# HandBrake/HandBrake

Measured on AMD Instinct MI355X. Metric: filtered frames/sec, 1080p YUV420p NLMeans+decomb chain, higher is better.
Workload: dtype u8 (f32 NLMeans weights, 16-bit fixed-point scaler as zimg, sharpen mix = the reference's f64 expression, as one f32 multiply where init proves that equal); 1 GPU; BASELINE configs[3]: decomb(31, EEDI2 bob) -> nlmeans medium -> cropscale lanczos 1920x1080 -> 3840x2160 -> lapsharp, 1080i YUV420P 8-bit in, inputs resident in HBM; input=1920x1080, output=3840x2160, streams_per_gpu=1, content=interlaced, stream_frames=48, stage_streams=2, parallelism=1 GPU(s) x 1 independent stream(s), device=AMD Radeon Graphics (gfx950:sramecc+:xnack-, 256 CUs)

## Files before the change

### handbrake_amd/csrc/decomb.hip

```cpp
#include "hbhip_internal.h"
#include "eedi2_engine.h"
#include <algorithm>
#include <vector>

namespace {

enum { M_YADIF = 1, M_BLEND = 2, M_CUBIC = 4, M_EEDI2 = 8, M_BOB = 16, M_SELECTIVE = 32 };
enum { PIC_TFF = 0x0008, PIC_PROGRESSIVE = 0x0010 };

struct DecombPlane
{
    const uint8_t *prev, *cur, *next, *guess;
    uint8_t       *dst;
    int            pitch, guess_pitch, dst_pitch, w, h;
};

struct DecombArgs
{
    DecombPlane pl[3];
    int mode;
    int parity;
    int field_parity;
};

// ... 5 lines not shown
__device__ __forceinline__ int max3i(int a, int b, int c) { return max(max(a, b), c); }
__device__ __forceinline__ int min3i(int a, int b, int c) { return min(min(a, b), c); }

constexpr int DB_FRAMES = 16;

struct DecombFrame
{
    const uint8_t *prev[3], *cur[3], *next[3], *guess[3];
    uint8_t       *dst[3];
    int mode, parity, field_parity, pad;
};

struct DecombBatch
{
    DecombFrame f[DB_FRAMES];
    int pitch[3], guess_pitch[3], dst_pitch[3], w[3], h[3];
    int n = 0;
    int ff = 0;
};

template <typename PIX> struct Px4;
template <> struct Px4<uint8_t>
{
    typedef uint32_t T;
    static __device__ __forceinline__ T zero() { return 0u; }
    static __device__ __forceinline__ int get(T v, int k) { return (int)((v >> (8 * k)) & 0xffu); }
    static __device__ __forceinline__ T pack(const int (&o)[4]) { return ((uint32_t)o[0] & 0xffu) | (((uint32_t)o[1] & 0xffu) << 8) | (((uint32_t)o[2] & 0xffu) << 16) | ((uint32_t)o[3] << 24); }
};
template <> struct Px4<uint16_t>
{
    typedef uint2 T;
    static __device__ __forceinline__ T zero() { return make_uint2(0u, 0u); }
    static __device__ __forceinline__ int get(T v, int k) { return (int)(((k < 2 ? v.x : v.y) >> (16 * (k & 1))) & 0xffffu); }
    static __device__ __forceinline__ T pack(const int (&o)[4]) { return make_uint2(((uint32_t)o[0] & 0xffffu) | ((uint32_t)o[1] << 16), ((uint32_t)o[2] & 0xffffu) | ((uint32_t)o[3] << 16)); }
};
template <typename PIX> struct W12 { typename Px4<PIX>::T w0, w1, w2; };

template <typename PIX>
__device__ __forceinline__ int w12b(const W12<PIX> &w, int i)
{
    const int k = i + 4;
    return Px4<PIX>::get(k < 4 ? w.w0 : (k < 8 ? w.w1 : w.w2), k & 3);
}

template <typename PIX>
__device__ __forceinline__ W12<PIX> ldw12(const uint8_t *row, int x, int pitch)
{
    typedef typename Px4<PIX>::T T;
    const T *p = reinterpret_cast<const T *>(row + (size_t)x * sizeof(PIX));
    return W12<PIX>{ x >= 4 ? p[-1] : Px4<PIX>::zero(), p[0], x + 4 < pitch ? p[1] : Px4<PIX>::zero() };
}

template <typename PIX>
__global__ __launch_bounds__(256) void decomb_plane4_kernel(DecombBatch B, int maxv)
{
    typedef Px4<PIX> X4;
    typedef typename X4::T T;
    typedef W12<PIX> WIN;
    const int pl = blockIdx.z % 3;
    const DecombFrame &F = B.f[blockIdx.z / 3];
    const int w = B.w[pl], h = B.h[pl], st = B.pitch[pl];
    const int pitch_s = st / (int)sizeof(PIX);
    const int x = 4 * (blockIdx.x * blockDim.x + threadIdx.x);
    const int y = blockIdx.y * blockDim.y + threadIdx.y;
    if (x >= w || y >= h) return;
    const uint8_t *cb = F.cur[pl];
    const uint8_t *crow = cb + (size_t)y * st;
    uint8_t *orow = F.dst[pl] + (size_t)y * B.dst_pitch[pl];
    const int mode = F.mode;
    auto store = [&](T v) {
        PIX *o = reinterpret_cast<PIX *>(orow) + x;
        if (x + 3 < w) *reinterpret_cast<T *>(o) = v;
        else for (int k = 0; k < 4 && x + k < w; k++) o[k] = (PIX)X4::get(v, k);
    };
    auto dw = [&](const uint8_t *row) { return *reinterpret_cast<const T *>(row + (size_t)x * sizeof(PIX)); };
    auto dwb = [](T v, int k) { return X4::get(v, k); };

    if (mode == 0) { store(dw(crow)); return; }
    if ((mode & M_EEDI2) && !(mode & M_YADIF))
    {
        store(dw(F.guess[pl] + (size_t)y * B.guess_pitch[pl]));
        return;
    }
    if ((y & 1) != (F.parity ? 0 : 1)) { store(dw(crow)); return; }

    int o4[4] = { 0, 0, 0, 0 };
    if (mode == M_BLEND)
    {
        int u1, u2, d1, d2;
        if (y > 1 && y < h - 2) { u1 = -st; u2 = -2 * st; d1 = st; d2 = 2 * st; }
        else if (y == 0)        { u1 = u2 = 0; d1 = st; d2 = 2 * st; }
        else if (y == 1)        { u1 = u2 = -st; d1 = st; d2 = 2 * st; }
        else if (y == h - 2)    { u1 = -st; u2 = -2 * st; d1 = d2 = st; }
        else                    { u1 = -st; u2 = -2 * st; d1 = d2 = 0; }
        const T a2 = dw(crow + u2), a1 = dw(crow + u1), c0 = dw(crow), b1 = dw(crow + d1), b2 = dw(crow + d2);
#pragma unroll
        for (int k = 0; k < 4; k++)
            o4[k] = cropv((-dwb(a2, k) + 2 * dwb(a1, k) + 6 * dwb(c0, k) + 2 * dwb(b1, k) - dwb(b2, k)) >> 3, maxv);
        store(X4::pack(o4));
        return;
    }
    if (mode == M_CUBIC)
    {
        int o0, o1, o2, o3;
        if (y >= 3)                { o0 = -3 * st; o1 = -st; }
        else if (y == 2 || y == 1) { o0 = o1 = -st; }
        else                       { o0 = o1 = st; }
        if (y <= h - 4)                    { o2 = st; o3 = 3 * st; }
        else if (y == h - 3 || y == h - 2) { o2 = o3 = st; }
        else                               { o2 = o3 = -st; }
        const T p0 = dw(crow + o0), p1 = dw(crow + o1), p2 = dw(crow + o2), p3 = dw(crow + o3);
#pragma unroll
        for (int k = 0; k < 4; k++) o4[k] = cubic4(dwb(p0, k), dwb(p1, k), dwb(p2, k), dwb(p3, k), maxv);
        store(X4::pack(o4));
        return;
    }
    if (!(mode & M_YADIF)) return;

// ... 48 lines not shown
        const int td2 = (abs(dwb(pnu, k) - cc) + abs(dwb(pnd, k) - e)) >> 1;
        int diff = max3i(td0 >> 1, td1, td2);
        int pred;
        if (!spatial) pred = dwb(g, k);
        else
        {
            pred = use_cubic ? cubic4(w12b(cu3, k), cc, e, w12b(cd3, k), maxv) : (cc + e) >> 1;
            const int xx = x + k;
            if (xx > margin && xx < w - (margin + 1))
            {
                auto slope = [&](int j) -> int {
                    if constexpr (sizeof(PIX) == 1)
                        return (int)__builtin_amdgcn_sad_u8(CU[3 + k + j], CD[3 + k - j], 0u);
                    else
                        return abs(w12b(cu, k - 1 + j) - w12b(cd, k - 1 - j)) + abs(w12b(cu, k + j) - w12b(cd, k - j)) +
                               abs(w12b(cu, k + 1 + j) - w12b(cd, k + 1 - j));
                };
                int best = slope(0) - 1;
                auto check = [&](int j) -> bool {
                    const int score = slope(j);
                    if (score >= best) return false;
                    best = score;
                    if (use_cubic)
                    {
                        if (j == -1)      pred = cubic4(w12b(cu3, k - 3), w12b(cu, k - 1), w12b(cd, k + 1), w12b(cd3, k + 3), maxv);
                        else if (j == -2) pred = cubic4((w12b(cu3, k - 4) + w12b(cu, k - 4)) / 2, w12b(cu, k - 2), w12b(cd, k + 2),
                                                        (w12b(cd3, k + 4) + w12b(cd, k + 4)) / 2, maxv);
                        else if (j == 1)  pred = cubic4(w12b(cu3, k + 3), w12b(cu, k + 1), w12b(cd, k - 1), w12b(cd3, k - 3), maxv);
                        else              pred = cubic4((w12b(cu3, k + 4) + w12b(cu, k + 4)) / 2, w12b(cu, k + 2), w12b(cd, k - 2),
                                                        (w12b(cd3, k - 4) + w12b(cd, k - 4)) / 2, maxv);
                    }
                    else pred = (w12b(cu, k + j) + w12b(cd, k - j)) >> 1;
                    return true;
                };
                if (check(-1)) check(-2);
                if (check(1)) check(2);
            }
        }
        if (!vertical_edge)
        {
            const int b = (dwb(p2a, k) + dwb(n2a, k)) >> 1;
            const int f = (dwb(p2b, k) + dwb(n2b, k)) >> 1;
            const int mx = max3i(d - e, d - cc, min(b - cc, f - e));
            const int mn = min3i(d - e, d - cc, max(b - cc, f - e));
            diff = max3i(diff, mn, -mx);
        }
        if (pred > d + diff)      pred = d + diff;
        else if (pred < d - diff) pred = d - diff;
        o4[k] = pred;
    }
    store(X4::pack(o4));
}


template <typename PIX>
__global__ __launch_bounds__(256) void bwdif_kernel(DecombArgs a, int field_end, int clip_max)
{
    typedef Px4<PIX> X4;
    typedef typename X4::T T;
    const DecombPlane &P = a.pl[blockIdx.z];
    const int x = 4 * (blockIdx.x * blockDim.x + threadIdx.x);
    const int y = blockIdx.y * blockDim.y + threadIdx.y;
    if (x >= P.w || y >= P.h) return;
    const int st = P.pitch, df = (int)sizeof(PIX), h = P.h;
    const uint8_t *cur = P.cur + (size_t)y * st;
    uint8_t *orow = P.dst + (size_t)y * P.dst_pitch;
    auto dw = [&](const uint8_t *row) { return *reinterpret_cast<const T *>(row + (size_t)x * sizeof(PIX)); };
    auto store = [&](T v) {
        PIX *o = reinterpret_cast<PIX *>(orow) + x;
        if (x + 3 < P.w) *reinterpret_cast<T *>(o) = v;
        else for (int k = 0; k < 4 && x + k < P.w; k++) o[k] = (PIX)X4::get(v, k);
    };
    if (a.mode == 0 || !((y ^ a.parity) & 1))
    {
        store(dw(cur));
        return;
    }
    constexpr int lf0 = 4309, lf1 = 213, hf0 = 5570, hf1 = 3801, hf2 = 1016, sp0 = 5077, sp1 = 981;
    int o4[4];
    if (field_end)
    {
        const int prefs = (y + df) < h ? st : -st, mrefs = y > (df - 1) ? -st : st;
        const int prefs3 = (y + 3 * df) < h ? 3 * st : -st, mrefs3 = y > (3 * df - 1) ? -3 * st : st;
        const T c1 = dw(cur + mrefs), e1 = dw(cur + prefs), c3 = dw(cur + mrefs3), e3 = dw(cur + prefs3);
#pragma unroll
        for (int k = 0; k < 4; k++)
        {
            const int v = (sp0 * (X4::get(c1, k) + X4::get(e1, k)) - sp1 * (X4::get(c3, k) + X4::get(e3, k))) >> 13;
            o4[k] = min(max(v, 0), clip_max);
        }
        store(X4::pack(o4));
        return;
    }
    const uint8_t *prev = P.prev + (size_t)y * st, *next = P.next + (size_t)y * st;
    const uint8_t *prev2 = a.field_parity ? prev : cur;
    const uint8_t *next2 = a.field_parity ? cur : next;
    const bool edge = (y < 4) || ((y + 5) > h);
    const int prefs = edge ? ((y + df) < h ? st : -st) : st, mrefs = edge ? (y > (df - 1) ? -st : st) : -st;
    const bool spat = edge ? !((y < 2) || ((y + 3) > h)) : true;
    const T wc = dw(cur + mrefs), we = dw(cur + prefs), wp0 = dw(prev2), wn0 = dw(next2);
    const T wpm = dw(prev + mrefs), wpp = dw(prev + prefs), wnm = dw(next + mrefs), wnp = dw(next + prefs);
    T wp2a = X4::zero(), wn2a = X4::zero(), wp2b = X4::zero(), wn2b = X4::zero();
    if (spat) { wp2a = dw(prev2 - 2 * st); wn2a = dw(next2 - 2 * st); wp2b = dw(prev2 + 2 * st); wn2b = dw(next2 + 2 * st); }
    T wc3a = X4::zero(), wc3b = X4::zero(), wp4a = X4::zero(), wn4a = X4::zero(), wp4b = X4::zero(), wn4b = X4::zero();
    if (!edge)
    {
// ... 171 lines not shown
        DecombArgs a;
        for (int c = 0; c < 3; c++)
        {
            DecombPlane &P = a.pl[c];
            P.prev = ref[0]->plane[c]; P.cur = ref[1]->plane[c]; P.next = ref[2]->plane[c];
            P.guess = nullptr; P.guess_pitch = 0;
            if ((mode & M_EEDI2) && eedi && slot >= 0)
            {
                const EediFrame g = eedi->result(slot);
                P.guess = g.plane[c];
                P.guess_pitch = g.stride[c];
            }
            P.dst = dst->plane[c];
            P.pitch = ref[1]->pitch[c]; P.dst_pitch = dst->pitch[c];
            P.w = in_geo.pw[c]; P.h = in_geo.ph[c];
        }
        a.mode = mode; a.parity = parity; a.field_parity = parity ^ tff;
        dim3 block(64, 4), grid((in_geo.pw[0] + 63) / 64, (in_geo.ph[0] + 3) / 4, 3);
        const int maxv = (1 << in_geo.depth) - 1;
        if (ff_bwdif)
        {
            if (bw_second && bw_field == BW_BACK_END) bw_field = BW_END;
            const int field_end = mode != 0 && bw_field == BW_END;
            const dim3 grid4(hbhip_grid_x((in_geo.pw[0] + 255) / 256), (in_geo.ph[0] + 3) / 4, 3);
            if (in_geo.bps == 2) HBHIP_LAUNCH(ctx, "bwdif", bwdif_kernel<uint16_t>, grid4, block, 0, a, field_end, maxv);
            else                 HBHIP_LAUNCH(ctx, "bwdif", bwdif_kernel<uint8_t>, grid4, block, 0, a, field_end, maxv);
            if (mode != 0 && bw_field == BW_END) bw_field = BW_NORMAL;
            HBHIP_CHECK(ctx, hipGetLastError());
            return HBHIP_OK;
        }
        geo.ff = ff_yadif ? (ff_nospatial ? 2 : 1) : 0;
        DecombFrame F;
        for (int c = 0; c < 3; c++)
        {
            const DecombPlane &P = a.pl[c];
            F.prev[c] = P.prev; F.cur[c] = P.cur; F.next[c] = P.next; F.guess[c] = P.guess; F.dst[c] = P.dst;
            geo.pitch[c] = P.pitch; geo.dst_pitch[c] = P.dst_pitch; geo.w[c] = P.w; geo.h[c] = P.h;
            if (P.guess) geo.guess_pitch[c] = P.guess_pitch;
        }
        F.mode = a.mode; F.parity = a.parity; F.field_parity = a.field_parity; F.pad = 0;
        gathered.push_back(F);
        return HBHIP_OK;
    }

    int launch_gathered(hbhip_ctx *lc)
    {
        for (size_t i0 = 0; i0 < gathered.size(); i0 += DB_FRAMES)
        {
            DecombBatch B = geo;
            B.n = (int)std::min<size_t>(DB_FRAMES, gathered.size() - i0);
            for (int k = 0; k < B.n; k++) B.f[k] = gathered[i0 + k];
            const dim3 block(64, 4), grid(hbhip_grid_x((B.w[0] + 255) / 256), (B.h[0] + 3) / 4, 3 * B.n);
            const int maxv = (1 << in_geo.depth) - 1;
            if (ff_yadif)
            {
                if (in_geo.bps == 2) HBHIP_LAUNCH(lc, "yadif", decomb_plane4_kernel<uint16_t>, grid, block, 0, B, maxv);
                else                 HBHIP_LAUNCH(lc, "yadif", decomb_plane4_kernel<uint8_t>, grid, block, 0, B, maxv);
            }
            else
            {
                if (in_geo.bps == 2) HBHIP_LAUNCH(lc, "decomb_plane", decomb_plane4_kernel<uint16_t>, grid, block, 0, B, maxv);
                else                 HBHIP_LAUNCH(lc, "decomb_plane", decomb_plane4_kernel<uint8_t>, grid, block, 0, B, maxv);
            }
        }
        const bool any = !gathered.empty();
        gathered.clear();
        if (any) HBHIP_CHECK(lc, hipGetLastError());
        return HBHIP_OK;
    }

    int process_frame()
    {
        DevPicture *cur = ref[1];
        const bool selective = par.mode & M_SELECTIVE;
        if (selective && cur->combed == 0)
        {
            DevPicture *o = pool.acquire();
            if (!o) return HBHIP_ERR_NOMEM;
            o->tag = cur->tag << 1; o->aux = 0;
            bw_second = false;
            int rc = launch(o, 0, 0, 0);
            if (rc != HBHIP_OK) return rc;
            outq.push_back(o);
            return HBHIP_OK;
        }
        int tff;
        if (par.parity < 0)
            tff = ff_yadif ? (cur->combed ? !!(cur->flags & PIC_TFF) : 1)
                           : (((cur->flags & PIC_PROGRESSIVE) == 0) ? !!(cur->flags & PIC_TFF) : 1);
        else
            tff = (par.parity & 1) ^ 1;

        const int is_combed = selective ? cur->combed : 2;
        int mode = 0;
        if ((par.mode & M_BLEND) && is_combed == 1) mode = M_BLEND;
        else if (is_combed != 0)                    mode = par.mode & ~M_SELECTIVE;

        const int nframes = (par.mode & M_BOB) ? 2 : 1;
        for (int frame = 0; frame < nframes; frame++)
        {
            const int parity = frame ^ tff ^ 1;
            int slot = -1;
            if ((mode & M_EEDI2) && eedi)
            {
                if (eedi->queued() == eedi->capacity())
                {
                    int rc = flush_batch();
// ... 140 lines not shown
```

### handbrake_amd/csrc/sharpen.hip

```cpp
#include <map>
#include <mutex>
#include <utility>
#include "hbhip_internal.h"

namespace {

struct LapKernel { int tap[25]; int size; double coef; };

constexpr LapKernel LAP_TABLE[4] = {
    { { 0, -1, 0, -1, 5, -1, 0, -1, 0 }, 3, 1.0 },
    { { -1, -4, -1, -4, 25, -4, -1, -4, -1 }, 3, 1.0 / 5 },
    { { 0, 0, -1, 0, 0, 0, -1, -2, -1, 0, -1, -2, 21, -2, -1, 0, -1, -2, -1, 0, 0, 0, -1, 0, 0 }, 5, 1.0 / 5 },
    { { 0, -1, -1, -1, 0, -1, -3, -4, -3, -1, -1, -4, 55, -4, -1, -1, -3, -4, -3, -1, 0, -1, -1, -1, 0 }, 5, 1.0 / 15 } };

struct LapArgs
{
    const uint8_t *src;
    uint8_t       *dst;
    int            width, height, src_pitch, dst_pitch;
    int            stride_border;
    int            valid_w;
    int            tap[25];
    double         coef, strength;
};

struct LapArgs3 { LapArgs p[3]; };

__device__ __forceinline__ uint32_t byte_at(const uint32_t (&v)[3], int k)
{
    const int kk = k + 4;
    return (v[kk >> 2] >> (8 * (kk & 3))) & 0xffu;
}

template <int S>
__global__ __launch_bounds__(256) void lapsharp_kernel(LapArgs3 all)
{
    const LapArgs &a = all.p[blockIdx.z];
    constexpr int LO = -((S - 1) / 2), HI = (S + 1) / 2;
    const int x0 = (blockIdx.x * blockDim.x + threadIdx.x) * 4;
    const int y = blockIdx.y;
    if (x0 >= a.width || y >= a.height) return;

    const int pitch_dw = a.src_pitch >> 2;
    const int xd = x0 >> 2;
    uint32_t rows[S][3];
#pragma unroll
    for (int j = 0; j < S; j++)
    {
        int yy = y + LO + j;
        yy = min(max(yy, 0), a.height - 1);
        const uint32_t *r = reinterpret_cast<const uint32_t *>(a.src + (size_t)yy * a.src_pitch);
        rows[j][0] = r[max(xd - 1, 0)];
        rows[j][1] = r[xd];
        rows[j][2] = r[min(xd + 1, pitch_dw - 1)];
        if (x0 + 8 > a.valid_w)
        {
// ... 409 lines not shown
            const uint32_t t = (uint32_t)tf;
            const int p = (int)((C[S] >> (8 * k)) & 0xffu);
            const int blur = (int)((t + (uint32_t)P.halfscale) >> P.scalebits);
            const int d = ((p - blur) * P.amount) >> 16;
            int res = B.sign > 0 ? p + d : p - d;
            res = res > B.vmax ? B.vmax : res < B.vmin ? B.vmin : res;
            packed |= (uint32_t)res << (8 * k);
        }
        store_row(y, packed);
#pragma unroll
        for (int j = 0; j < NT - 1; j++)
        {
            C[j] = C[j + 1];
#pragma unroll
            for (int k = 0; k < 4; k++) H[j][k] = H[j + 1][k];
        }
    }
}

__global__ void plane_copy_kernel(uint8_t *dst, int dst_pitch, const uint8_t *src, int src_pitch,
                                  int row_bytes, int rows)
{
    const int x = (blockIdx.x * blockDim.x + threadIdx.x) * 4;
    const int y = blockIdx.y;
    if (y >= rows || x >= row_bytes) return;
    const uint8_t *s = src + (size_t)y * src_pitch + x;
    uint8_t *d = dst + (size_t)y * dst_pitch + x;
    if (x + 3 < row_bytes)
        *reinterpret_cast<uint32_t *>(d) = *reinterpret_cast<const uint32_t *>(s);
    else
        for (int i = 0; x + i < row_bytes; i++) d[i] = s[i];
}

int launch_copy(hbhip_ctx *ctx, const char *name, DevPicture *in, DevPicture *out, int c)
{
    const int row = in->width[c] * in->bps;
    dim3 grid((row / 4 + 255) / 256 + 1, in->height[c]);
    HBHIP_LAUNCH(ctx, name, plane_copy_kernel, grid, dim3(256), 0, out->plane[c], out->pitch[c],
                 (const uint8_t *)in->plane[c], in->pitch[c], row, in->height[c]);
    HBHIP_CHECK(ctx, hipGetLastError());
    return HBHIP_OK;
}

#ifndef LS_ROWS_N
#define LS_ROWS_N 8
#endif
#ifndef LS_BX_N
#define LS_BX_N 64
#endif
#ifndef LS_ROWS16_N
#define LS_ROWS16_N 4
#endif
constexpr int LS_ROWS = LS_ROWS_N, LS_ROWS16 = LS_ROWS16_N, LS_FRAMES = 16, LS_BX = LS_BX_N, LS_BY = 256 / LS_BX_N;
struct LapPlane3 { int width, height, src_pitch, dst_pitch, stride_border, valid_w, a, b, c, active; double coef, strength; int fast, kinv; float mixf; };
struct LapBatch3
{
    LapPlane3      pl[3];
    const uint8_t *src[LS_FRAMES][3];
    uint8_t       *dst[LS_FRAMES][3];
};

__global__ __launch_bounds__(256) void lapsharp3_rows_kernel(LapBatch3 B)
{
    const int job = blockIdx.z, f = job / 3, c = job - 3 * f;
    const LapPlane3 &P = B.pl[c];
    if (!P.active) return;
    const int x0 = (blockIdx.x * LS_BX + threadIdx.x) * 4;
    const int ys = (blockIdx.y * LS_BY + threadIdx.y) * LS_ROWS;
    if (x0 >= P.width || ys >= P.height) return;
    const uint8_t *src = B.src[f][c];
    uint8_t *dst = B.dst[f][c];
    const int pitch_dw = P.src_pitch >> 2, xd = x0 >> 2;
    const bool tail = x0 + 8 > P.valid_w;

    int u_prev[4], u_cur[4], v_cur[4], m_cur[4];
    const uint32_t o0 = 4u * (uint32_t)max(xd - 1, 0), o1 = 4u * (uint32_t)xd, o2 = 4u * (uint32_t)min(xd + 1, pitch_dw - 1);
    uint32_t raw[LS_ROWS + 2][3];
#pragma unroll
    for (int i = 0; i < LS_ROWS + 2; i++)
    {
        const int yy = min(max(ys - 1 + i, 0), P.height - 1);
        const uint32_t ro = (uint32_t)__mul24(yy, P.src_pitch);
        raw[i][0] = *reinterpret_cast<const uint32_t *>(src + (ro + o0));
        raw[i][1] = *reinterpret_cast<const uint32_t *>(src + (ro + o1));
        raw[i][2] = *reinterpret_cast<const uint32_t *>(src + (ro + o2));
    }
    auto load_row = [&](int i, int (&u)[4], int (&v)[4], int (&m)[4]) {
        uint32_t w[3] = { raw[i][0], raw[i][1], raw[i][2] };
        if (tail)
        {
#pragma unroll
            for (int k = 0; k < 3; k++)
            {
                const int keep = P.valid_w - (x0 - 4 + 4 * k);
                if (keep <= 0) w[k] = 0;
                else if (keep < 4) w[k] &= (1u << (8 * keep)) - 1u;
            }
        }
        const int b_1 = (int)(w[0] >> 24), b0 = (int)(w[1] & 0xff), b1 = (int)((w[1] >> 8) & 0xff),
                  b2 = (int)((w[1] >> 16) & 0xff), b3 = (int)(w[1] >> 24), b4 = (int)(w[2] & 0xff);
        const int bb[6] = { b_1, b0, b1, b2, b3, b4 };
#pragma unroll
        for (int k = 0; k < 4; k++)
        {
            const int h = bb[k] + bb[k + 2];
            m[k] = bb[k + 1];
            u[k] = __mul24(P.a, h) + __mul24(P.b, m[k]);
// ... 14 lines not shown
#pragma unroll
    for (int r = 0; r < LS_ROWS; r++)
    {
        const int y = ys + r;
        if (y >= y_end) break;
        int u_next[4], v_next[4], m_next[4];
        load_row(r + 2, u_next, v_next, m_next);
        const bool row_copy = (y < 2) || (y > P.height - 2);
        uint32_t packed = 0;
        if (row_copy)
        {
#pragma unroll
            for (int k = 0; k < 4; k++) packed |= (uint32_t)m_cur[k] << (8 * k);
        }
        else
        {
            if (P.fast)
            {
#pragma unroll
                for (int k = 0; k < 4; k++)
                {
                    const int centre = m_cur[k];
                    const int acc = u_prev[k] + v_cur[k] + u_next[k];
                    int out = (int)((float)(acc - __mul24(P.kinv, centre)) * P.mixf) + centre;
                    out = min(max(out, 0), 255);
                    packed |= (uint32_t)out << (8 * k);
                }
            }
            else
            {
#pragma unroll
                for (int k = 0; k < 4; k++)
                {
                    const int centre = m_cur[k];
                    const int acc = u_prev[k] + v_cur[k] + u_next[k];
                    const double mixed = (((double)acc * P.coef) - (double)centre) * P.strength;
                    int out = (int)(short)(int)mixed + centre;
                    out = min(max(out, 0), 255);
                    packed |= (uint32_t)out << (8 * k);
                }
            }
            if (copy_cols)
            {
#pragma unroll
                for (int k = 0; k < 4; k++)
                    if ((copy_cols >> k) & 1u) packed = (packed & ~(0xffu << (8 * k))) | ((uint32_t)m_cur[k] << (8 * k));
            }
        }
        uint8_t *d = dst + ((uint32_t)__mul24(y, P.dst_pitch) + (uint32_t)x0);
        if (full_dword) *reinterpret_cast<uint32_t *>(d) = packed;
        else for (int k = 0; x0 + k < P.width; k++) d[k] = (uint8_t)(packed >> (8 * k));
#pragma unroll
        for (int k = 0; k < 4; k++) { u_prev[k] = u_cur[k]; u_cur[k] = u_next[k]; v_cur[k] = v_next[k]; m_cur[k] = m_next[k]; }
    }
}

__global__ __launch_bounds__(256) void lapsharp3_rows16_kernel(LapBatch3 B, int max_value)
{
    const int job = blockIdx.z, f = job / 3, c = job - 3 * f;
    const LapPlane3 &P = B.pl[c];
    if (!P.active) return;
    const int x0 = (blockIdx.x * LS_BX + threadIdx.x) * 4;
    const int ys = (blockIdx.y * LS_BY + threadIdx.y) * LS_ROWS16;
    if (x0 >= P.width || ys >= P.height) return;
    const uint8_t *src = B.src[f][c];
    uint8_t *dst = B.dst[f][c];
    const int pitch_dw = P.src_pitch >> 2, xd = x0 >> 1;
    const bool tail = x0 + 5 > P.width;
    const uint32_t o0 = 4u * (uint32_t)max(xd - 1, 0), o1 = 4u * (uint32_t)xd, o2 = 4u * (uint32_t)min(xd + 1, pitch_dw - 1),
                   o3 = 4u * (uint32_t)min(xd + 2, pitch_dw - 1);
    int u_prev[4], u_cur[4], v_cur[4], m_cur[4];
    uint32_t raw[LS_ROWS16 + 2][4];
#pragma unroll
    for (int i = 0; i < LS_ROWS16 + 2; i++)
    {
        const uint32_t ro = (uint32_t)__mul24(min(max(ys - 1 + i, 0), P.height - 1), P.src_pitch);
        raw[i][0] = *reinterpret_cast<const uint32_t *>(src + (ro + o0)); raw[i][1] = *reinterpret_cast<const uint32_t *>(src + (ro + o1));
        raw[i][2] = *reinterpret_cast<const uint32_t *>(src + (ro + o2)); raw[i][3] = *reinterpret_cast<const uint32_t *>(src + (ro + o3));
    }
    auto load_row = [&](int i, int (&u)[4], int (&v)[4], int (&m)[4]) {
        const uint32_t ro = (uint32_t)__mul24(min(max(ys - 1 + i, 0), P.height - 1), P.src_pitch);
        const uint32_t w0 = raw[i][0], w1 = raw[i][1], w2 = raw[i][2], w3 = raw[i][3];
        int bb[6] = { (int)(w0 >> 16), (int)(w1 & 0xffffu), (int)(w1 >> 16), (int)(w2 & 0xffffu), (int)(w2 >> 16), (int)(w3 & 0xffffu) };
        if (tail)
        {
            const uint16_t *r16 = reinterpret_cast<const uint16_t *>(src + ro);
#pragma unroll
            for (int k = 0; k < 6; k++)
            {
                const int xx = x0 - 1 + k;
                if (xx >= P.width) bb[k] = (int)r16[max(2 * P.width - 1 - xx, 0)];
            }
        }
#pragma unroll
        for (int k = 0; k < 4; k++)
        {
            const int h = bb[k] + bb[k + 2];
            m[k] = bb[k + 1];
            u[k] = __mul24(P.a, h) + __mul24(P.b, m[k]);
            v[k] = __mul24(P.b, h) + __mul24(P.c, m[k]);
        }
    };
    {
        int v_tmp[4], m_tmp[4];
        load_row(0, u_prev, v_tmp, m_tmp);
        load_row(1, u_cur, v_cur, m_cur);
// ... 54 lines not shown
                if ((int)(short)(int)mixed != (int)prod) { ok = false; break; }
            }
        if (ok) { kinv = ki; mixf = c; return true; }
    }
    return false;
}

static bool lap_float_mix_cached(int kernel, double strength, int &kinv, float &mixf)
{
    struct Entry { bool ok; int kinv; float mixf; };
    static std::mutex lock;
    static std::map<std::pair<int, double>, Entry> cache;
    std::lock_guard<std::mutex> lk(lock);
    const auto key = std::make_pair(kernel, strength);
    auto it = cache.find(key);
    if (it == cache.end())
    {
        Entry e = { false, 0, 0.f };
        e.ok = lap_float_mix(LAP_TABLE[kernel], strength, e.kinv, e.mixf);
        it = cache.emplace(key, e).first;
    }
    kinv = it->second.kinv;
    mixf = it->second.mixf;
    return it->second.ok;
}

class LapsharpFilter : public BurstFilter
{
public:
    LapsharpFilter(hbhip_ctx *c, const hbhip_lapsharp_params &p) : BurstFilter(c), par(p)
    {
        for (int pl = 0; pl < 3; pl++)
        {
            mix_fast[pl] = LAP_TABLE[par.kernel[pl]].size == 3 && lap_float_mix_cached(par.kernel[pl], par.strength[pl], mix_k[pl], mix_f[pl]);
            rows3 &= LAP_TABLE[par.kernel[pl]].size == 3;
        }
    }
    template <class P>
    void fill_plane(P &p, const DevPicture *in, const DevPicture *out, int c) const
    {
        p.width = in->width[c]; p.height = in->height[c];
        p.src_pitch = in->pitch[c]; p.dst_pitch = out->pitch[c];
        const int hb_stride = in_is_dev ? hbhip_align_up(in->width[c] * in->bps, 64) / in->bps : in_stride[c] / in->bps;
        p.stride_border = (hb_stride - in->width[c]) / 2;
        p.valid_w = in_is_dev ? in->width[c] : (1 << 30);
        p.coef = LAP_TABLE[par.kernel[c]].coef; p.strength = par.strength[c];
    }
    int process_many(DevPicture *const *ins, DevPicture *const *outs, int n) override
    {
        return hbhip_for_each_run(ctx, ins, outs, n, LS_FRAMES, [&](int at, int nf) {
            if (!rows3) return hbhip_each_frame(ins, outs, at, nf, [&](DevPicture *in, DevPicture *out) { return one_frame(in, out); });
            LapBatch3 B;
            int max_w = 0, max_h = 0;
            for (int c = 0; c < 3; c++)
            {
                const LapKernel &k = LAP_TABLE[par.kernel[c]];
                LapPlane3 &P = B.pl[c];
                fill_plane(P, ins[at], outs[at], c);
                P.a = k.tap[0]; P.b = k.tap[1]; P.c = k.tap[4];
                P.active = 1;
                P.fast = in_geo.bps == 1 && mix_fast[c]; P.kinv = mix_k[c]; P.mixf = mix_f[c];
                max_w = std::max(max_w, P.width); max_h = std::max(max_h, P.height);
                for (int f = 0; f < nf; f++)
                {
                    B.src[f][c] = ins[at + f]->plane[c];
                    B.dst[f][c] = outs[at + f]->plane[c];
                }
            }
            const int rows = LS_BY * (in_geo.bps == 1 ? LS_ROWS : LS_ROWS16);
            const dim3 grid(hbhip_grid_x(((max_w + 3) / 4 + LS_BX - 1) / LS_BX), (max_h + rows - 1) / rows, 3 * nf);
            if (in_geo.bps == 1) HBHIP_LAUNCH(ctx, "lapsharp_3x3", lapsharp3_rows_kernel, grid, dim3(LS_BX, LS_BY), 0, B);
            else                 HBHIP_LAUNCH(ctx, "lapsharp_3x3", lapsharp3_rows16_kernel, grid, dim3(LS_BX, LS_BY), 0, B, (1 << in_geo.depth) - 1);
            return HBHIP_OK;
        });
    }
    int one_frame(DevPicture *in, DevPicture *out)
    {
        for (int size : {3, 5})
        {
            LapArgs3 all;
            int n = 0, max_w = 0, max_h = 0;
            for (int c = 0; c < 3; c++)
            {
                const LapKernel &k = LAP_TABLE[par.kernel[c]];
                if (k.size != size) continue;
                LapArgs &a = all.p[n++];
                a.src = in->plane[c]; a.dst = out->plane[c];
                fill_plane(a, in, out, c);
                for (int i = 0; i < 25; i++) a.tap[i] = k.tap[i];
                max_w = std::max(max_w, a.width); max_h = std::max(max_h, a.height);
            }
            if (n == 0) continue;
            const char *name = size == 3 ? "lapsharp_3x3" : "lapsharp_5x5";
            if (in->bps == 2)
            {
                const dim3 grid(((max_w + 1) / 2 + 255) / 256, max_h, n);
                const int max_value = (1 << in_geo.depth) - 1;
                if (size == 3) HBHIP_LAUNCH(ctx, name, lapsharp16_kernel<3>, grid, dim3(256), 0, all, max_value);
                else           HBHIP_LAUNCH(ctx, name, lapsharp16_kernel<5>, grid, dim3(256), 0, all, max_value);
            }
            else
            {
                const dim3 grid(((max_w + 3) / 4 + 255) / 256, max_h, n);
                if (size == 3) HBHIP_LAUNCH(ctx, name, lapsharp_kernel<3>, grid, dim3(256), 0, all);
                else           HBHIP_LAUNCH(ctx, name, lapsharp_kernel<5>, grid, dim3(256), 0, all);
            }
        }
        return HBHIP_OK;
    }
    hbhip_lapsharp_params par;
    bool  rows3 = true;
    bool  mix_fast[3] = {};
    int   mix_k[3] = {};
    float mix_f[3] = {};
};

static void binomial_row(int steps, uint32_t *coef, int len)
{
    for (int i = 0; i < len; i++) coef[i] = 0;
    coef[0] = 1;
// ... 148 lines not shown
```

Measured before the change: 9792 output frames/s.

## Add row-walking decomb EEDI2+yadif kernel and wide DPP/udot4 lapsharp kernel

Adds a decomb kernel where each thread walks several field rows of the EEDI2+yadif path, keeping cur/prev/next and temporal rows in registers and also writing the copied field line. This cuts redundant global loads and per-row setup. Separately, adds a wide 3x3 lapsharp kernel that covers 8 pixels per thread, shares horizontal neighbours across lanes via DPP, and computes row sums with udot4/alignbyte. Both are gated by runtime checks (8-bit input, tap signs, alignment) and fall back to the old kernels otherwise. The price is higher register pressure and fewer threads in flight.

```diff
diff --git a/handbrake_amd/csrc/decomb.hip b/handbrake_amd/csrc/decomb.hip
--- a/handbrake_amd/csrc/decomb.hip
+++ b/handbrake_amd/csrc/decomb.hip
@@ -81,18 +81,13 @@
 }
 
 template <typename PIX>
-__global__ __launch_bounds__(256) void decomb_plane4_kernel(DecombBatch B, int maxv)
+__device__ __forceinline__ void decomb_row4(const DecombBatch &B, const DecombFrame &F, int pl, int x, int y, int maxv)
 {
     typedef Px4<PIX> X4;
     typedef typename X4::T T;
     typedef W12<PIX> WIN;
-    const int pl = blockIdx.z % 3;
-    const DecombFrame &F = B.f[blockIdx.z / 3];
     const int w = B.w[pl], h = B.h[pl], st = B.pitch[pl];
     const int pitch_s = st / (int)sizeof(PIX);
-    const int x = 4 * (blockIdx.x * blockDim.x + threadIdx.x);
-    const int y = blockIdx.y * blockDim.y + threadIdx.y;
-    if (x >= w || y >= h) return;
     const uint8_t *cb = F.cur[pl];
     const uint8_t *crow = cb + (size_t)y * st;
     uint8_t *orow = F.dst[pl] + (size_t)y * B.dst_pitch[pl];
@@ -247,6 +242,95 @@
     store(X4::pack(o4));
 }
 
+template <typename PIX>
+__global__ __launch_bounds__(256) void decomb_plane4_kernel(DecombBatch B, int maxv)
+{
+    const int pl = blockIdx.z % 3;
+    const int x = 4 * (blockIdx.x * blockDim.x + threadIdx.x);
+    const int y = blockIdx.y * blockDim.y + threadIdx.y;
+    if (x >= B.w[pl] || y >= B.h[pl]) return;
+    decomb_row4<PIX>(B, B.f[blockIdx.z / 3], pl, x, y, maxv);
+}
+
+#ifndef DW_R_N
+#define DW_R_N 8
+#endif
+constexpr int DW_R = DW_R_N;
+
+__global__ __launch_bounds__(256) void decomb_rowwalk8_kernel(DecombBatch B, int maxv)
+{
+    typedef Px4<uint8_t> X4;
+    const int pl = blockIdx.z % 3;
+    const DecombFrame &F = B.f[blockIdx.z / 3];
+    const int w = B.w[pl], h = B.h[pl], st = B.pitch[pl], dst_st = B.dst_pitch[pl];
+    const int x = 4 * (blockIdx.x * blockDim.x + threadIdx.x);
+    const int ys = (blockIdx.y * blockDim.y + threadIdx.y) * (2 * DW_R);
+    if (x >= w || ys >= h) return;
+    const int y0 = ys + (F.parity ? 0 : 1);
+    const bool walk = (F.mode & M_EEDI2) && (F.mode & M_YADIF) && !B.ff && y0 >= 3 && y0 + 2 * (DW_R - 1) <= h - 4;
+    if (!walk)
+    {
+        for (int r = 0; r < 2 * DW_R && ys + r < h; r++) decomb_row4<uint8_t>(B, F, pl, x, ys + r, maxv);
+        return;
+    }
+    auto dw = [&](const uint8_t *base, int y, int pitch) { return *reinterpret_cast<const uint32_t *>(base + (size_t)y * pitch + x); };
+    auto store = [&](int y, uint32_t v) {
+        uint8_t *o = F.dst[pl] + (size_t)y * dst_st + x;
+        if (x + 3 < w) *reinterpret_cast<uint32_t *>(o) = v;
+        else for (int k = 0; k < 4 && x + k < w; k++) o[k] = (uint8_t)X4::get(v, k);
+    };
+    const uint8_t *p2base = F.field_parity ? F.prev[pl] : F.cur[pl], *n2base = F.field_parity ? F.cur[pl] : F.next[pl];
+    uint32_t cu[DW_R + 1], pv[DW_R + 1], nx[DW_R + 1], p2[DW_R + 2], n2[DW_R + 2], gs[DW_R];
+#pragma unroll
+    for (int i = 0; i < DW_R + 1; i++)
+    {
+        cu[i] = dw(F.cur[pl], y0 - 1 + 2 * i, st); pv[i] = dw(F.prev[pl], y0 - 1 + 2 * i, st); nx[i] = dw(F.next[pl], y0 - 1 + 2 * i, st);
+    }
+#pragma unroll
+    for (int i = 0; i < DW_R + 2; i++) { p2[i] = dw(p2base, y0 - 2 + 2 * i, st); n2[i] = dw(n2base, y0 - 2 + 2 * i, st); }
+#pragma unroll
+    for (int i = 0; i < DW_R; i++) gs[i] = dw(F.guess[pl], y0 + 2 * i, B.guess_pitch[pl]);
+
+    int cc[4], a_pu[4], a_nu[4], b[4], d[4], td0[4];
+#pragma unroll
+    for (int k = 0; k < 4; k++)
+    {
+        cc[k] = X4::get(cu[0], k);
+        a_pu[k] = abs(X4::get(pv[0], k) - cc[k]);
+        a_nu[k] = abs(X4::get(nx[0], k) - cc[k]);
+        b[k] = (X4::get(p2[0], k) + X4::get(n2[0], k)) >> 1;
+        d[k] = (X4::get(p2[1], k) + X4::get(n2[1], k)) >> 1;
+        td0[k] = abs(X4::get(p2[1], k) - X4::get(n2[1], k));
+    }
+#pragma unroll
+    for (int i = 0; i < DW_R; i++)
+    {
+        const int y = y0 + 2 * i;
+        int o4[4];
+#pragma unroll
+        for (int k = 0; k < 4; k++)
+        {
+            const int e = X4::get(cu[i + 1], k);
+            const int a_pd = abs(X4::get(pv[i + 1], k) - e), a_nd = abs(X4::get(nx[i + 1], k) - e);
+            const int P2 = X4::get(p2[i + 2], k), N2 = X4::get(n2[i + 2], k);
+            const int f = (P2 + N2) >> 1;
+            const int td1 = (a_pu[k] + a_pd) >> 1, td2 = (a_nu[k] + a_nd) >> 1;
+            int diff = max3i(td0[k] >> 1, td1, td2);
+            int pred = X4::get(gs[i], k);
+            const int mx = max3i(d[k] - e, d[k] - cc[k], min(b[k] - cc[k], f - e));
+            const int mn = min3i(d[k] - e, d[k] - cc[k], max(b[k] - cc[k], f - e));
+            diff = max3i(diff, mn, -mx);
+            if (pred > d[k] + diff)      pred = d[k] + diff;
+            else if (pred < d[k] - diff) pred = d[k] - diff;
+            o4[k] = pred;
+            cc[k] = e; a_pu[k] = a_pd; a_nu[k] = a_nd; b[k] = d[k]; d[k] = f; td0[k] = abs(P2 - N2);
+        }
+        store(y, X4::pack(o4));
+        if (F.parity) store(y + 1, cu[i + 1]);
+        else          store(y - 1, cu[i]);
+    }
+}
+
 
 template <typename PIX>
 __global__ __launch_bounds__(256) void bwdif_kernel(DecombArgs a, int field_end, int clip_max)
@@ -524,7 +608,14 @@
             for (int k = 0; k < B.n; k++) B.f[k] = gathered[i0 + k];
             const dim3 block(64, 4), grid(hbhip_grid_x((B.w[0] + 255) / 256), (B.h[0] + 3) / 4, 3 * B.n);
             const int maxv = (1 << in_geo.depth) - 1;
-            if (ff_yadif)
+            bool walk = !ff_yadif && in_geo.bps == 1;
+            for (int k = 0; k < B.n; k++) walk &= (B.f[k].mode & M_EEDI2) && (B.f[k].mode & M_YADIF) && B.f[k].guess[0];
+            if (walk)
+            {
+                const dim3 wgrid(grid.x, (B.h[0] + 8 * DW_R - 1) / (8 * DW_R), grid.z);
+                HBHIP_LAUNCH(lc, "decomb_plane", decomb_rowwalk8_kernel, wgrid, block, 0, B, maxv);
+            }
+            else if (ff_yadif)
             {
                 if (in_geo.bps == 2) HBHIP_LAUNCH(lc, "yadif", decomb_plane4_kernel<uint16_t>, grid, block, 0, B, maxv);
                 else                 HBHIP_LAUNCH(lc, "yadif", decomb_plane4_kernel<uint8_t>, grid, block, 0, B, maxv);
diff --git a/handbrake_amd/csrc/lapsharp_rowdot.h b/handbrake_amd/csrc/lapsharp_rowdot.h
--- /dev/null
+++ b/handbrake_amd/csrc/lapsharp_rowdot.h
@@ -0,0 +1,62 @@
+#pragma once
+#include <hip/hip_runtime.h>
+#include <cstdint>
+
+#define LRD_FN __host__ __device__ __forceinline__
+
+LRD_FN uint32_t lrd_alignbyte(uint32_t hi, uint32_t lo, int sh)
+{
+#if defined(__HIP_DEVICE_COMPILE__)
+    return __builtin_amdgcn_alignbyte(hi, lo, (uint32_t)sh);
+#else
+    return (uint32_t)(((((uint64_t)hi) << 32) | lo) >> (8 * sh));
+#endif
+}
+
+LRD_FN uint32_t lrd_udot4(uint32_t x, uint32_t taps, uint32_t acc)
+{
+#if defined(__HIP_DEVICE_COMPILE__)
+    return __builtin_amdgcn_udot4(x, taps, acc, false);
+#else
+    for (int k = 0; k < 4; k++) acc += ((x >> (8 * k)) & 0xffu) * ((taps >> (8 * k)) & 0xffu);
+    return acc;
+#endif
+}
+
+struct LrdTaps { uint32_t tu, th; int c; };
+LRD_FN bool lrd_taps(int a, int b, int c, LrdTaps &t)
+{
+    if (a > 0 || b > 0 || c < 0 || a < -255 || b < -255 || c > 255) return false;
+    const uint32_t ma = (uint32_t)-a, mb = (uint32_t)-b;
+    t.tu = ma | (mb << 8) | (ma << 16);
+    t.th = mb | (mb << 16);
+    t.c = c;
+    return true;
+}
+
+template <int NDW>
+LRD_FN uint32_t lrd_window(const uint32_t (&ext)[NDW + 2], int p)
+{
+    const int o = 3 + p;
+    return (o & 3) ? lrd_alignbyte(ext[(o >> 2) + 1], ext[o >> 2], o & 3) : ext[o >> 2];
+}
+
+LRD_FN uint32_t lrd_row_u(uint32_t win, const LrdTaps &t) { return lrd_udot4(win, t.tu, 0u); }
+LRD_FN uint32_t lrd_row_h(uint32_t win, const LrdTaps &t) { return lrd_udot4(win, t.th, 0u); }
+LRD_FN uint32_t lrd_neg_sum(uint32_t h_own, uint32_t u_above, uint32_t u_below) { return h_own + u_above + u_below; }
+LRD_FN int lrd_acc(int centre, uint32_t n, const LrdTaps &t) { return t.c * centre - (int)n; }
+
+template <int K>
+LRD_FN float lrd_mix_fast(uint32_t own, uint32_t n, float ckf, float mixf)
+{
+    const float fm = (float)((own >> (8 * K)) & 0xffu);
+#if defined(__HIP_DEVICE_COMPILE__)
+    const float t = __builtin_fmaf(ckf, fm, -(float)n);
+    return __builtin_truncf(t * mixf) + fm;
+#else
+    const float t = __builtin_fmaf(ckf, fm, -(float)n);
+    const volatile float prod = t * mixf;
+    return __builtin_truncf(prod) + fm;
+#endif
+}
+LRD_FN uint32_t lrd_sat_u8(float v) { return v <= 0.f ? 0u : v >= 255.f ? 255u : (uint32_t)v; }
diff --git a/handbrake_amd/csrc/sharpen.hip b/handbrake_amd/csrc/sharpen.hip
--- a/handbrake_amd/csrc/sharpen.hip
+++ b/handbrake_amd/csrc/sharpen.hip
@@ -2,6 +2,7 @@
 #include <mutex>
 #include <utility>
 #include "hbhip_internal.h"
+#include "lapsharp_rowdot.h"
 
 namespace {
 
@@ -517,7 +518,7 @@
 #define LS_ROWS16_N 4
 #endif
 constexpr int LS_ROWS = LS_ROWS_N, LS_ROWS16 = LS_ROWS16_N, LS_FRAMES = 16, LS_BX = LS_BX_N, LS_BY = 256 / LS_BX_N;
-struct LapPlane3 { int width, height, src_pitch, dst_pitch, stride_border, valid_w, a, b, c, active; double coef, strength; int fast, kinv; float mixf; };
+struct LapPlane3 { int width, height, src_pitch, dst_pitch, stride_border, valid_w, a, b, c, active; double coef, strength; int fast, kinv; float mixf; LrdTaps taps; float ckf; };
 struct LapBatch3
 {
     LapPlane3      pl[3];
@@ -638,6 +639,165 @@
         else for (int k = 0; x0 + k < P.width; k++) d[k] = (uint8_t)(packed >> (8 * k));
 #pragma unroll
         for (int k = 0; k < 4; k++) { u_prev[k] = u_cur[k]; u_cur[k] = u_next[k]; v_cur[k] = v_next[k]; m_cur[k] = m_next[k]; }
+    }
+}
+
+#ifndef LW_DW_N
+#define LW_DW_N 2
+#endif
+#ifndef LW_WX_N
+#define LW_WX_N 2
+#endif
+#ifndef LW_BY_N
+#define LW_BY_N 2
+#endif
+#ifndef LW_ROWS_N
+#define LW_ROWS_N 8
+#endif
+constexpr int LW_DW = LW_DW_N, LW_WX = LW_WX_N, LW_BY = LW_BY_N, LW_ROWS = LW_ROWS_N;
+constexpr int LW_PX = 4 * LW_DW, LW_WAVE_SPAN = 64 * LW_PX, LW_SPAN = LW_WX * LW_WAVE_SPAN;
+struct alignas(4 * LW_DW) LwVec { uint32_t v[LW_DW]; };
+
+__device__ __forceinline__ uint32_t lw_from_lane_below(uint32_t x)
+{
+    return (uint32_t)__builtin_amdgcn_update_dpp(0, (int)x, 0x138 , 0xf, 0xf, false);
+}
+__device__ __forceinline__ uint32_t lw_from_lane_above(uint32_t x)
+{
+    return (uint32_t)__builtin_amdgcn_update_dpp(0, (int)x, 0x130 , 0xf, 0xf, false);
+}
+__device__ __forceinline__ uint32_t lw_keep_mask(int keep) { return keep <= 0 ? 0u : keep >= 4 ? 0xffffffffu : (1u << (8 * keep)) - 1u; }
+
+__global__ __launch_bounds__(64 * LW_WX * LW_BY) void lapsharp3_wide_kernel(LapBatch3 B)
+{
+    constexpr int NDW = LW_DW, PX = LW_PX, R = LW_ROWS;
+    const int job = blockIdx.z, f = job / 3, c = job - 3 * f;
+    const LapPlane3 &P = B.pl[c];
+    if (!P.active) return;
+    const int lane = threadIdx.x & 63;
+    const int x0 = (blockIdx.x * (64 * LW_WX) + threadIdx.x) * PX;
+    const int ys = (blockIdx.y * LW_BY + threadIdx.y) * R;
+    const int wave_x0 = x0 - lane * PX;
+    if (wave_x0 >= P.width || ys >= P.height) return;
+    const uint8_t *src = B.src[f][c];
+    uint8_t *dst = B.dst[f][c];
+    const uint32_t ow = (uint32_t)min(x0, P.src_pitch - PX);
+    const bool rclamp = x0 + PX >= P.src_pitch;
+    const bool lload = lane == 0, rload = lane == 63 && !rclamp;
+    const uint32_t oe = (uint32_t)min(lload ? max(x0 - 4, 0) : x0 + PX, P.src_pitch - 4);
+    const bool tail = wave_x0 + LW_WAVE_SPAN + 4 > P.valid_w;
+    uint32_t keep[NDW + 2];
+#pragma unroll
+    for (int j = 0; j < NDW + 2; j++) keep[j] = lw_keep_mask(P.valid_w - (x0 - 4 + 4 * j));
+
+    LwVec raw[R + 2];
+    uint32_t edge[R + 2];
+#pragma unroll
+    for (int i = 0; i < R + 2; i++)
+    {
+        const int yy = min(max(ys - 1 + i, 0), P.height - 1);
+        raw[i] = *reinterpret_cast<const LwVec *>(src + ((uint32_t)__mul24(yy, P.src_pitch) + ow));
+        edge[i] = 0;
+    }
+    if (lload || rload)
+    {
+#pragma unroll
+        for (int i = 0; i < R + 2; i++)
+        {
+            const int yy = min(max(ys - 1 + i, 0), P.height - 1);
+            edge[i] = *reinterpret_cast<const uint32_t *>(src + ((uint32_t)__mul24(yy, P.src_pitch) + oe));
+        }
+    }
+    const LrdTaps taps = P.taps;
+    auto prep = [&](int i, uint32_t (&u)[PX], uint32_t (&h)[PX]) __attribute__((always_inline)) {
+        const uint32_t below = lw_from_lane_below(raw[i].v[NDW - 1]), above = lw_from_lane_above(raw[i].v[0]);
+        uint32_t ext[NDW + 2];
+        ext[0] = lload ? edge[i] : below;
+#pragma unroll
+        for (int k = 0; k < NDW; k++) ext[1 + k] = raw[i].v[k];
+        ext[NDW + 1] = rclamp ? raw[i].v[NDW - 1] : rload ? edge[i] : above;
+        if (tail)
+        {
+#pragma unroll
+            for (int j = 0; j < NDW + 2; j++) ext[j] &= keep[j];
+#pragma unroll
+            for (int k = 0; k < NDW; k++) raw[i].v[k] = ext[1 + k];
+        }
+#pragma unroll
+        for (int p = 0; p < PX; p++)
+        {
+            const uint32_t win = lrd_window<NDW>(ext, p);
+            u[p] = lrd_row_u(win, taps);
+            h[p] = lrd_row_h(win, taps);
+        }
+    };
+    uint32_t u_prev[PX], u_cur[PX], h_cur[PX];
+    {
+        uint32_t h_tmp[PX];
+        prep(0, u_prev, h_tmp);
+        prep(1, u_cur, h_cur);
+    }
+    uint32_t copy_cols[NDW];
+    bool has_copy = false;
+#pragma unroll
+    for (int k = 0; k < NDW; k++)
+    {
+        copy_cols[k] = 0;
+#pragma unroll
+        for (int j = 0; j < 4; j++)
+            if (x0 + 4 * k + j < P.stride_border + 2 || x0 + 4 * k + j > P.width + P.stride_border - 2) copy_cols[k] |= 0xffu << (8 * j);
+        has_copy |= copy_cols[k] != 0;
+    }
+    const int y_end = min(ys + R, P.height);
+    const float ckf = P.ckf, mixf = P.mixf;
+#pragma unroll
+    for (int r = 0; r < R; r++)
+    {
+        const int y = ys + r;
+        if (y >= y_end) break;
+        uint32_t u_next[PX], h_next[PX];
+        prep(r + 2, u_next, h_next);
+        const LwVec own = raw[r + 1];
+        LwVec out = own;
+        if (!((y < 2) || (y > P.height - 2)))
+        {
+#pragma unroll
+            for (int k = 0; k < NDW; k++)
+            {
+                uint32_t packed = 0;
+                if (P.fast)
+                {
+#define LW_PIX(J) packed = __builtin_amdgcn_cvt_pk_u8_f32(lrd_mix_fast<J>(own.v[k], lrd_neg_sum(h_cur[4 * k + J], u_prev[4 * k + J], u_next[4 * k + J]), ckf, mixf), J, packed)
+                    LW_PIX(0); LW_PIX(1); LW_PIX(2); LW_PIX(3);
+#undef LW_PIX
+                }
+                else
+                {
+#pragma unroll
+                    for (int j = 0; j < 4; j++)
+                    {
+                        const int centre = (int)((own.v[k] >> (8 * j)) & 0xffu);
+                        const int acc = lrd_acc(centre, lrd_neg_sum(h_cur[4 * k + j], u_prev[4 * k + j], u_next[4 * k + j]), taps);
+                        const double mixed = (((double)acc * P.coef) - (double)centre) * P.strength;
+                        int o = (int)(short)(int)mixed + centre;
+                        o = min(max(o, 0), 255);
+                        packed |= (uint32_t)o << (8 * j);
+                    }
+                }
+                if (has_copy) packed = (packed & ~copy_cols[k]) | (own.v[k] & copy_cols[k]);
+                out.v[k] = packed;
+            }
+        }
+        uint8_t *d = dst + ((uint32_t)__mul24(y, P.dst_pitch) + (uint32_t)x0);
+        if (x0 + PX <= P.width) *reinterpret_cast<LwVec *>(d) = out;
+        else
+        {
+#pragma unroll
+            for (int k = 0; k < PX; k++)
+                if (x0 + k < P.width) d[k] = (uint8_t)(out.v[k >> 2] >> (8 * (k & 3)));
+        }
+#pragma unroll
+        for (int p = 0; p < PX; p++) { u_prev[p] = u_cur[p]; u_cur[p] = u_next[p]; h_cur[p] = h_next[p]; }
     }
 }
 
@@ -798,6 +958,8 @@
             if (!rows3) return hbhip_each_frame(ins, outs, at, nf, [&](DevPicture *in, DevPicture *out) { return one_frame(in, out); });
             LapBatch3 B;
             int max_w = 0, max_h = 0;
+            bool wide = in_geo.bps == 1;
+            uintptr_t bits = 0;
             for (int c = 0; c < 3; c++)
             {
                 const LapKernel &k = LAP_TABLE[par.kernel[c]];
@@ -806,12 +968,23 @@
                 P.a = k.tap[0]; P.b = k.tap[1]; P.c = k.tap[4];
                 P.active = 1;
                 P.fast = in_geo.bps == 1 && mix_fast[c]; P.kinv = mix_k[c]; P.mixf = mix_f[c];
+                wide &= lrd_taps(P.a, P.b, P.c, P.taps) && P.src_pitch >= LW_PX;
+                P.ckf = (float)(P.c - P.kinv);
+                bits |= (uintptr_t)(P.src_pitch | P.dst_pitch);
                 max_w = std::max(max_w, P.width); max_h = std::max(max_h, P.height);
                 for (int f = 0; f < nf; f++)
                 {
                     B.src[f][c] = ins[at + f]->plane[c];
                     B.dst[f][c] = outs[at + f]->plane[c];
+                    bits |= (uintptr_t)B.src[f][c] | (uintptr_t)B.dst[f][c];
                 }
+            }
+            wide &= (bits & (4 * LW_DW - 1)) == 0 && max_w >= LW_WAVE_SPAN;
+            if (wide)
+            {
+                const dim3 grid(hbhip_grid_x((max_w + LW_SPAN - 1) / LW_SPAN), (max_h + LW_BY * LW_ROWS - 1) / (LW_BY * LW_ROWS), 3 * nf);
+                HBHIP_LAUNCH(ctx, "lapsharp_3x3", lapsharp3_wide_kernel, grid, dim3(64 * LW_WX, LW_BY), 0, B);
+                return HBHIP_OK;
             }
             const int rows = LS_BY * (in_geo.bps == 1 ? LS_ROWS : LS_ROWS16);
             const dim3 grid(hbhip_grid_x(((max_w + 3) / 4 + LS_BX - 1) / LS_BX), (max_h + rows - 1) / rows, 3 * nf);
```

New measurement: 10050 output frames/s (median of 6 runs). 2.6% higher.
